# YaqiXia/Voltrix-SpMM

Hardware: AMD Instinct MI355X
Metric: spmm_gflops (higher is better)
Workload: dtype f16

## Files before the change

### voltrix-spmm_amd/voltrix/hybrid.py

```python
from __future__ import annotations

import contextlib
import contextvars
import dataclasses
import os

import torch

from . import capi

DEFAULT_WAVES = 8
DEFAULT_ROW_BLOCKS = 4
DEFAULT_TAU = 3
KSTEP = 32
FUSED_WAVES = 4
FUSED_ROW_BLOCKS = 8


@dataclasses.dataclass
class PanelParts:
    parts: torch.Tensor
    cuts: torch.Tensor
    xcd_ptr: torch.Tensor
    max_parts_per_xcd: int
# ... 11 lines not shown
    panel_order: torch.Tensor
    num_nodes: int
    waves: int
    row_blocks: int
    tau: int
    num_ksteps: int
    num_shared_edges: int
    num_resid_edges: int
    xcd_ptr: torch.Tensor = None
    max_panels_per_xcd: int = 0
    parts: PanelParts = None

    @property
    def panel_rows(self) -> int:
        return self.waves * self.row_blocks * 16

    @property
    def num_panels(self) -> int:
        return (self.num_nodes + self.panel_rows - 1) // self.panel_rows


@dataclasses.dataclass(eq=False)
class TwoLevelHandle:
    blk_offsets: torch.Tensor
    hspa_packed: torch.Tensor
    hind: torch.Tensor
    plan: PanelPlan
    num_nodes: int
    num_edges: int
    hash_tag: str = None
    fused: "FusedRecords" = None
    window_xcd_ptr: torch.Tensor = None
    format_choice: dict = dataclasses.field(default_factory=dict)

    @property
    def residual(self):
        return self.blk_offsets, self.hspa_packed, self.hind


@dataclasses.dataclass
class FusedRecords:
    wave_ptr: torch.Tensor
    records: torch.Tensor
    num_records: int

    def nbytes(self) -> int:
        return self.wave_ptr.numel() * 4 + self.records.numel() * 4


RECORD_WORDS = 64


def build_fused_records_torch(blk_offsets: torch.Tensor, hspa_packed: torch.Tensor, hind: torch.Tensor, num_nodes: int,
                              waves: int = FUSED_WAVES, row_blocks: int = FUSED_ROW_BLOCKS) -> FusedRecords:
    assert blk_offsets.dtype == torch.int32 and hind.dtype == torch.int32 and hspa_packed.dtype == torch.uint32
    device = blk_offsets.device
    num_windows = (num_nodes + 15) // 16
    panel_rows = waves * row_blocks * 16
    num_waves = waves * ((num_nodes + panel_rows - 1) // panel_rows)
    bo = blk_offsets.to(torch.int64)
    kb0, kb1 = bo[:-1], bo[1:]
    nblk = kb1 - kb0
    packed = hspa_packed.view(torch.int32).view(-1, 4)
    hind64 = hind
    total_blocks = packed.shape[0]
    zero_first = (packed[kb0.clamp(max=max(total_blocks - 1, 0))] == 0).all(dim=1) if total_blocks else nblk < 0
# ... 65 lines not shown
    resid_indptr[1:] = torch.cumsum(torch.bincount(resid_rows, minlength=n), 0)
    new_index = torch.cumsum(shared_u.to(torch.int64), 0) - 1
    sk = key[shared_e]
    return (resid_indptr.to(torch.int32), resid_indices, uniq[shared_u], sk % p, new_index[inverse[shared_e]])


MAX_PLAN_COLS = 1 << 22
MAX_PLAN_EDGE_PASSES = 2 * 10 ** 10


def canonical_csr(indptr: torch.Tensor, indices: torch.Tensor, num_nodes: int, num_cols: int):
    deg = (indptr[1:] - indptr[:-1]).to(torch.int64)
    rows = torch.repeat_interleave(torch.arange(num_nodes, device=indptr.device, dtype=torch.int64), deg)
    key = torch.unique(rows * num_cols + indices.to(torch.int64), sorted=True)
    rows = key // num_cols
    out_indptr = torch.zeros(num_nodes + 1, dtype=torch.int64, device=indptr.device)
    out_indptr[1:] = torch.cumsum(torch.bincount(rows, minlength=num_nodes), 0)
    return out_indptr.to(torch.int32), (key - rows * num_cols).to(torch.int32)


def empty_plan(num_nodes, waves, row_blocks, tau, device, num_edges):
    np_ = (num_nodes + waves * row_blocks * 16 - 1) // (waves * row_blocks * 16)
    return PanelPlan(panel_ptr=torch.zeros(np_ + 1, dtype=torch.int32, device=device),
                     panel_cols=torch.zeros(2 * KSTEP, dtype=torch.int32, device=device),
                     panel_bits=torch.zeros(waves * 64, dtype=torch.int32, device=device).view(torch.uint32),
                     panel_order=None, num_nodes=num_nodes, waves=waves, row_blocks=row_blocks, tau=tau, num_ksteps=0,
                     num_shared_edges=0, num_resid_edges=num_edges)


KSTEP_COST_IN_STAGES = 6.6
KSTEP_COST_X10 = 66


def balance_xcd_ranges(two: "TwoLevelHandle") -> None:
    plan = two.plan
    if plan.num_ksteps == 0 or plan.num_panels < 2 * 8:
        return
    cost_x10 = max(1, KSTEP_COST_X10 * plan.panel_rows // 512)
    if plan.panel_ptr.is_cuda:
        xcd_ptr, two.window_xcd_ptr = capi.xcd_ranges_of_panels(plan.panel_ptr, two.blk_offsets, two.num_nodes, plan.panel_rows,
                                                                cost_x10)
    else:
        xcd_ptr, two.window_xcd_ptr = xcd_ranges_of_panels_torch(plan.panel_ptr, two.blk_offsets, two.num_nodes,
                                                                 plan.panel_rows, cost_x10)
    longest_range, longest_panel = torch.stack([(xcd_ptr[1:] - xcd_ptr[:-1]).max(),
                                                (plan.panel_ptr[1:] - plan.panel_ptr[:-1]).max()]).tolist()
    plan.xcd_ptr = xcd_ptr
    plan.max_panels_per_xcd = int(longest_range)
    plan.panel_order = longest_first_order(plan.panel_ptr, xcd_ptr=xcd_ptr)
    cap = default_part_cap(plan.num_ksteps)
    if PANEL_PART_FACTOR > 0 and longest_panel > cap:
        plan.parts = panel_parts(plan.panel_ptr, cap, xcd_ptr)


def xcd_ranges_of_panels_torch(panel_ptr: torch.Tensor, resid_blk_offsets: torch.Tensor, num_nodes: int, panel_rows: int,
                               kstep_cost_x10: int):
    from .schedule import split_equal_work

    dev = panel_ptr.device
    num_panels = panel_ptr.numel() - 1
    windows_per_panel = panel_rows // 16
    num_windows = (num_nodes + 15) // 16
    nst = ((resid_blk_offsets[1:num_windows + 1] - resid_blk_offsets[:num_windows]).to(torch.int64) + 3) // 4
    pad = num_panels * windows_per_panel - num_windows
    stages = torch.cat([nst, torch.zeros(pad, dtype=torch.int64, device=dev)]).view(num_panels, windows_per_panel).sum(1)
    tenths = (panel_ptr[1:] - panel_ptr[:-1]).to(torch.int64) * kstep_cost_x10
    q, r = tenths // 10, tenths % 10
    q = q + ((r > 5) | ((r == 5) & (q % 2 == 1))).to(torch.int64)
    xcd_ptr = split_equal_work(q + stages)
    return xcd_ptr, (xcd_ptr.to(torch.int64) * windows_per_panel).clamp(max=num_windows).to(torch.int32)


PANEL_PART_FACTOR = 1.0
NUM_CUS = 256


def default_part_cap(num_ksteps: int) -> int:
    return max(32, int(PANEL_PART_FACTOR * num_ksteps / NUM_CUS))


def panel_parts(panel_ptr: torch.Tensor, cap: int, panel_xcd_ptr: torch.Tensor = None) -> PanelParts:
    if not panel_ptr.is_cuda:
        return panel_parts_torch(panel_ptr, cap, panel_xcd_ptr)
# ... 142 lines not shown
    bits = torch.zeros((total_ksteps + 1) * waves * 64, dtype=torch.int64, device=device)
    bits.index_add_(0, word, torch.ones_like(word) << (16 * (k % 2) + 4 * j + (k % 8) // 2))
    panel_bits = ((bits + 2 ** 31) % 2 ** 32 - 2 ** 31).to(torch.int32).view(torch.uint32)

    plan = PanelPlan(panel_ptr=panel_ptr.to(torch.int32), panel_cols=panel_cols.to(torch.int32), panel_bits=panel_bits,
                     panel_order=None, num_nodes=num_nodes, waves=waves, row_blocks=row_blocks, tau=tau,
                     num_ksteps=total_ksteps, num_shared_edges=int(rp.numel()),
                     num_resid_edges=int(resid_indices.numel()))
    return resid_indptr, resid_indices, plan


KSTEPS_PIPELINED = 17


def default_panel_tile(embedding_dim: int, waves: int, row_blocks: int = DEFAULT_ROW_BLOCKS):
    if embedding_dim <= 32:
        return (32, 6, 2)
    if embedding_dim <= 64:
        return (64, 6, 2)
    if waves == 8:
        return (128, 3, 1) if row_blocks == 4 else (128, 4, KSTEPS_PIPELINED)
    return (128, 4, 1)


PANEL_DOMINATED_RATIO = 2.0
PANEL_DOMINATED_ROW_BLOCKS = 2


def panel_dominated(plan: "PanelPlan") -> bool:
    resid_stages = max(1.0, plan.num_resid_edges / 32.0)
    return plan.num_ksteps * KSTEP_COST_IN_STAGES >= PANEL_DOMINATED_RATIO * resid_stages


_SIDE_STREAMS = {}


def side_stream(device) -> "torch.cuda.Stream":
    key = device.index if device.index is not None else torch.cuda.current_device()
    if key not in _SIDE_STREAMS:
        _SIDE_STREAMS[key] = torch.cuda.Stream(device=device)
    return _SIDE_STREAMS[key]


def run_two_level(plan: PanelPlan, operand: torch.Tensor, output: torch.Tensor, run_window, out_scale=None,
                  tile=None, concurrent: bool = True) -> None:
    def finish(pending):
        if pending is not None:
            pending.run()

    if plan.num_ksteps == 0:
        finish(run_window(False))
        return
    if not concurrent:
        finish(run_window(False))
        launch_panel(plan, operand, output, accumulate=1, out_scale=out_scale, tile=tile)
        return
    from .utils import timed_launch

    main = torch.cuda.current_stream()
    side = side_stream(operand.device)
    with timed_launch("zero_fill", main):
        output.zero_()
    fork = torch.cuda.Event()
    fork.record(main)
    side.wait_event(fork)
    pending_panel = launch_panel(plan, operand, output, accumulate=2, out_scale=out_scale, tile=tile,
                                 stream=side.cuda_stream, defer_combine=True)
    join = torch.cuda.Event()
    join.record(side)
    pending = run_window(True)
    main.wait_event(join)
    finish(pending)
    finish(pending_panel)


class PendingPanelCombine:

    def __init__(self, plan, partials, output, num_feats, accumulate):
        self.plan, self.partials, self.output, self.num_feats, self.accumulate = plan, partials, output, num_feats, accumulate

    def run(self, raw_stream: int = None):
        from .utils import timed_launch

        current = torch.cuda.current_stream()
        with timed_launch("combine_panel_partials", current) if raw_stream is None else contextlib.nullcontext():
            rc = capi.launch_combine_panel_partials(self.plan.parts, self.partials.data_ptr(), self.output.data_ptr(),
                                                    self.plan.num_nodes, self.num_feats, self.plan.panel_rows,
                                                    self.accumulate, current.cuda_stream if raw_stream is None else raw_stream)
        capi.check(rc, "voltrix_launch_combine_panel_partials")
        self.partials = None


def launch_panel(plan: PanelPlan, feat: torch.Tensor, output: torch.Tensor, accumulate, out_scale=None,
# ... 104 lines not shown
```

### voltrix-spmm_amd/voltrix/include/voltrix/spmm_kernels.hpp

```cpp
#pragma once

#include <hip/hip_runtime.h>

#include <cstdint>
#include <cstdlib>
#include <mutex>
#include <type_traits>
#include <utility>
#include <vector>

#include "voltrix/traits.hpp"

#ifndef VOLTRIX_DIAG
#define VOLTRIX_DIAG 0
#endif


namespace voltrix {

typedef _Float16 half8_t __attribute__((ext_vector_type(8)));
typedef __bf16 bf16x8_t __attribute__((ext_vector_type(8)));
typedef uint16_t bfloat16_bits;
typedef float float4_t __attribute__((ext_vector_type(4)));
typedef unsigned uint2_t __attribute__((ext_vector_type(2)));
// ... 183 lines not shown
    }
  if (hipFuncSetAttribute(kernel, hipFuncAttributeMaxDynamicSharedMemorySize, bytes) != hipSuccess) return kErrBadConfig;
  seen.push_back(Seen{kernel, dev});
  last = seen.back();
  return kOk;
}

template <class T>
struct SpmmArgs {
  using in_t = typename std::conditional<T::EB == 4, float,
                                         typename std::conditional<T::BF16, bfloat16_bits, _Float16>::type>::type;
  const int* blk_offsets;
  const uint32_t* hspa_packed;
  const int* hind;
  const in_t* input;
  float* output;
  int num_nodes;
  int num_windows;
  int F;
  int num_slabs;
  int windows_per_xcd;
  const int* window_order;
  const float* out_scale;
  const int4* units;
  const int* unit_ptr;
  float* partials;
  const in_t* values;
  const int* row_map;
  int slab_major;
  int slab_first;
  int meta_nt;
  int atomic_out;
};

template <int I, int N, class Fn>
__device__ __forceinline__ void static_for(Fn&& fn) {
  if constexpr (I < N) {
    fn(std::integral_constant<int, I>{});
    static_for<I + 1, N>(fn);
  }
}

template <class T, int NU>
__device__ __forceinline__ void spmm_tc16_body(const SpmmArgs<T>& a) {
  static_assert(NU == 1 || NU == 2, "units per wave");
  constexpr int FS = T::FS, D = T::DEPTH, MS = T::META_SLOTS, EB = T::EB;
  constexpr int ROW_BYTES = T::ROW_BYTES, STAGE_BYTES = T::STAGE_BYTES, NDMA = T::DMA_PER_STAGE;
  constexpr int RPD = T::ROWS_PER_DMA, LPR = T::LANES_PER_ROW, SLOTS = T::SLOTS;

  extern __shared__ __attribute__((aligned(16))) char smem[];
  const int lane = threadIdx.x & (kWave - 1);
  const int wave = __builtin_amdgcn_readfirstlane((int)(threadIdx.x / kWave));
  const unsigned long long diag_t0 = (VOLTRIX_DIAG & 8) ? __builtin_amdgcn_s_memrealtime() : 0ull;

  const int xcd = blockIdx.x % kNumXcd;
  int w_begin = xcd * a.windows_per_xcd;
  int w_count = (a.num_windows - w_begin) < a.windows_per_xcd ? (a.num_windows - w_begin) : a.windows_per_xcd;
  if (a.units) {
    w_begin = a.unit_ptr[xcd];
    w_count = a.unit_ptr[xcd + 1] - w_begin;
  }
  __builtin_amdgcn_s_setprio(3);
  const int wave_pos = (int)(blockIdx.x / kNumXcd) * T::WAVES + wave;
  const int pairs_per_slab = (w_count + 1) / 2;
  if (w_count <= 0 || (NU == 1 ? wave_pos >= w_count * a.num_slabs : wave_pos >= pairs_per_slab * a.num_slabs)) return;
  const int lu = NU == 1 ? wave_pos : (wave_pos / pairs_per_slab) * w_count + 2 * (wave_pos % pairs_per_slab);
// ... 340 lines not shown
    wait_vmcnt<0>();
  }

  if (VOLTRIX_DIAG & 4) {
    if (acc[0][0][0] == 12345.678f) a.output[0] = acc[0][0][0];
    return;
  }
  const float oscale = ((EB == 2 && !T::WEIGHTED) ? kAScaleInv : 1.0f) * (a.out_scale ? *a.out_scale : 1.0f);
  const int ocol0 = fs0 + (lane & 15);
#pragma unroll
  for (int p = 0; p < NU; ++p) {
    if (!present[p]) continue;
    const bool dead = NU > 1 && nst_u[p] == 0;
    if (slot[p] >= 0) {
      float* const tile = a.partials + (long long)slot[p] * (kBlkH * (long long)F) + (long long)(4 * (lane >> 4)) * F;
#pragma unroll
      for (int s = 0; s < SLOTS; ++s) {
        const int col = ocol0 + 16 * s;
        if (col < F) {
#pragma unroll
          for (int j = 0; j < 4; ++j) tile[(long long)j * F + col] = dead ? 0.f : acc[p][s][j] * oscale;
        }
      }
      continue;
    }
    const int orow0 = w[p] * kBlkH + 4 * (lane >> 4);
    int orow[4];
#pragma unroll
    for (int j = 0; j < 4; ++j) {
      orow[j] = orow0 + j;
      if (a.row_map && !(VOLTRIX_DIAG & 8)) orow[j] = a.row_map[orow[j]];
      if (orow[j] >= a.num_nodes) orow[j] = -1;
    }
#pragma unroll
    for (int s = 0; s < SLOTS; ++s) {
      const int col = ocol0 + 16 * s;
      if (col < F) {
#pragma unroll
        for (int j = 0; j < 4; ++j) {
          const int row = orow[j];
          if (row >= 0) {
            float* const dst = a.output + ((long long)row * F + col);
            const float v = dead ? 0.f : acc[p][s][j] * oscale;
            if (a.atomic_out)
              unsafeAtomicAdd(dst, v);
            else
              *dst = v;
          }
        }
      }
    }
  }
  if ((VOLTRIX_DIAG & 8) && a.row_map && lane == 0) {
    int* const stamp = const_cast<int*>(a.row_map) + 4ll * ((long long)blockIdx.x * T::WAVES + wave);
    stamp[0] = (int)__builtin_amdgcn_s_getreg((31 << 11) | 20);
    stamp[1] = (int)__builtin_amdgcn_s_getreg((31 << 11) | 4);
    stamp[2] = (int)(unsigned)diag_t0;
    stamp[3] = (int)(unsigned)__builtin_amdgcn_s_memrealtime();
  }
}

template <class T>
static __global__ __launch_bounds__(T::THREADS) void spmm_tc16_kernel(const SpmmArgs<T> a) {
  spmm_tc16_body<T, 1>(a);
}

template <class T>
static __global__ __launch_bounds__(T::THREADS) __attribute__((amdgpu_num_vgpr(160)))
void spmm_tc16_pair_kernel(const SpmmArgs<T> a) {
  spmm_tc16_body<T, 2>(a);
}

inline int slab_major_order(int num_slabs, int slab_row_bytes) { return num_slabs > 1 && slab_row_bytes >= 128; }

enum SlabPolicy : int { kSlabAuto = -1, kSlabOneGrid = 0, kSlabLaunches = 1 };
inline int slab_launch_group(int num_slabs, int slab_row_bytes, long long rows, int policy = kSlabAuto) {
  if (policy == kSlabOneGrid || slab_row_bytes < 128) return 0;
  if (policy == kSlabAuto && rows * 256 > (256ll << 20)) return 0;
  const int group = slab_row_bytes >= 256 ? 1 : 256 / slab_row_bytes;
  return num_slabs > group ? group : 0;
}

template <class T>
inline int launch_spmm_tc16(const int* blk_offsets, const uint32_t* hspa_packed, const int* hind, int num_nodes,
                            int embedding_dim, const void* input ,
                            float* output, hipStream_t stream, const int* window_order = nullptr,
                            const float* out_scale = nullptr, int atomic_out = 0,
                            const int* units = nullptr , const int* unit_ptr = nullptr ,
                            int max_units_per_xcd = 0, float* partials = nullptr, const int* row_map = nullptr,
                            const void* values = nullptr ,
                            int units_per_wave = 1 ,
                            int slab_first = 0, int slab_count = 0 ,
                            long long input_rows = 0 ,
                            int slab_policy = kSlabAuto) {
  if (num_nodes < 0 || embedding_dim < 0) return kErrBadShape;
  if (num_nodes == 0 || embedding_dim == 0) return kOk;
  if (embedding_dim % (16 / T::EB) != 0) return kErrBadShape;
  if (((uintptr_t)input & 15) || ((uintptr_t)hspa_packed & 15)) return kErrBadShape;
  SpmmArgs<T> a;
  a.blk_offsets = blk_offsets;
  a.hspa_packed = hspa_packed;
  a.hind = hind;
  a.input = static_cast<const typename SpmmArgs<T>::in_t*>(input);
  a.output = output;
  a.num_nodes = num_nodes;
  a.num_windows = (num_nodes + kBlkH - 1) / kBlkH;
  a.F = embedding_dim;
  const int total_slabs = (embedding_dim + T::FS - 1) / T::FS;
  if (slab_first < 0 || slab_count < 0 || slab_first + slab_count > total_slabs) return kErrBadShape;
  if (const int group = slab_count == 0 ? slab_launch_group(total_slabs, T::FS * T::EB,
                                                            input_rows > 0 ? input_rows : (long long)num_nodes, slab_policy)
                                        : 0) {
    for (int s = 0; s < total_slabs; s += group) {
      const int rc = launch_spmm_tc16<T>(blk_offsets, hspa_packed, hind, num_nodes, embedding_dim, input, output, stream,
                                         window_order, out_scale, atomic_out, units, unit_ptr, max_units_per_xcd, partials,
                                         row_map, values, units_per_wave, s, total_slabs - s < group ? total_slabs - s : group);
      if (rc != kOk) return rc;
    }
    return kOk;
  }
  a.slab_first = slab_count > 0 ? slab_first : 0;
  a.num_slabs = slab_count > 0 ? slab_count : total_slabs;
  a.windows_per_xcd = (a.num_windows + kNumXcd - 1) / kNumXcd;
  a.window_order = window_order;
  a.out_scale = out_scale;
  a.atomic_out = atomic_out;
  a.meta_nt = total_slabs == 1;
  a.slab_major = slab_major_order(a.num_slabs, T::FS * T::EB);
// ... 309 lines not shown
```

### voltrix-spmm_amd/voltrix/jit_kernels/spmm.py

```python
import contextlib
import contextvars
import ctypes
import os
import warnings
from typing import Callable, NamedTuple

import torch

from ..jit.compiler import hash_to_hex
from ..jit.template import map_ctype
from ..project import TUNE_SPACE_FLAG
from ..schedule import balanced_xcd_windows, default_max_stages, stream_tables, unit_table
from .tuner import jit_tuner

_TUNE_SPACE_OVERRIDE = contextvars.ContextVar("voltrix_tune_space", default=None)


def tune_space_mode() -> str:
    return _TUNE_SPACE_OVERRIDE.get() or os.getenv(TUNE_SPACE_FLAG, "default")


@contextlib.contextmanager
def tune_space(mode: str):
    token = _TUNE_SPACE_OVERRIDE.set(mode)
    try:
        yield
    finally:
        _TUNE_SPACE_OVERRIDE.reset(token)


includes = ('"voltrix/spmm_kernels.hpp"', '"voltrix/spmm_stream_kernels.hpp"')
template = """
if ({SCHED} == 6) {
  __return_code = voltrix::launch_spmm_stream<voltrix::SpmmTile<{FS}, {DEPTH}, {WAVES}, {EB}, {BF16} != 0, {WEIGHTED} != 0>>(
      hspa_packed, hind, num_nodes, embedding_dim, input, output, stream, s_units, s_runs, s_run_ptr, s_max_runs, partials_s,
      out_scale, 0, 0, input_rows, slab_policy);
  if (__return_code == 0 && combine_now != 0)
    __return_code = voltrix::combine_partials(cuts_s, num_cuts_s, partials_s, output, num_nodes, embedding_dim, 0, stream, nullptr);
  return;
}
__return_code = voltrix::launch_spmm_tc16<voltrix::SpmmTile<{FS}, {DEPTH}, {WAVES}, {EB}, {BF16} != 0, {WEIGHTED} != 0>>(
    blk_offsets, hspa_packed, hind,
    num_nodes, embedding_dim, input, output, stream,
    ({SCHED} == 0 || {SCHED} >= 4) ? nullptr : ({SCHED} == 1 ? win_order_a : ({SCHED} == 2 ? win_order_b : win_order_c)),
    out_scale, atomic_out,
    {SCHED} == 4 ? units : ({SCHED} == 5 ? units_p : nullptr), {SCHED} == 5 ? unit_ptr_p : unit_ptr,
    {SCHED} == 5 ? max_units_per_xcd_p : max_units_per_xcd, {SCHED} == 5 ? partials_p : partials,
    has_row_map != 0 ? row_map : nullptr, {WEIGHTED} != 0 ? (const void*)values : nullptr, {SCHED} == 5 ? 2 : 1,
    0, 0, input_rows, slab_policy);
if (__return_code == 0 && {SCHED} == 4 && combine_now != 0)
  __return_code = voltrix::combine_partials(cuts, num_cuts, partials, output, num_nodes, embedding_dim, atomic_out, stream,
                                            has_row_map != 0 ? row_map : nullptr);
if (__return_code == 0 && {SCHED} == 5 && combine_now != 0)
  __return_code = voltrix::combine_partials(cuts_p, num_cuts_p, partials_p, output, num_nodes, embedding_dim, atomic_out,
                                            stream, has_row_map != 0 ? row_map : nullptr);
"""

ORDER_CHUNKS = {1: 128, 2: 512, 3: 2048}
SCHED_UNITS = 4
SCHED_PAIRS = 5
SCHED_STREAM = 6
STREAM_MAX_BLOCKS_PER_WINDOW = 48
PAIR_UNIT_FACTOR = 1.25

SLAB_POLICY = -1


def slab_launches(embedding_dim: int, fs: int, elem_bytes: int, rows: int, policy: int = None) -> int:
    policy = SLAB_POLICY if policy is None else policy
    slabs = -(-embedding_dim // fs)
    slab_bytes = fs * elem_bytes
    if slab_bytes < 128 or policy == 0 or (policy < 0 and rows * 256 > (256 << 20)):
        return 1
    group = 1 if slab_bytes >= 256 else 256 // slab_bytes
    return -(-slabs // group) if slabs > group else 1


def feature_hash(feature: torch.Tensor) -> str:
    if hasattr(feature, "hash_tag") and isinstance(feature.hash_tag, str):
        return hash_to_hex(feature.hash_tag)
    warnings.warn(
        "The feature tensor(i.e. `hspa_packed`)'s hash_tag attr is not set. "
        "Voltrix will use the memory address as the key value for profiling, "
        "which may lead to performance degradation of different cases."
    )
    return hash_to_hex(str(feature.data_ptr()))

# ... 196 lines not shown
        ("win_order_b", torch.int32),
        ("win_order_c", torch.int32),
        ("out_scale", torch.float32),
        ("atomic_out", int),
        ("units", torch.int32),
        ("unit_ptr", torch.int32),
        ("max_units_per_xcd", int),
        ("cuts", torch.int32),
        ("num_cuts", int),
        ("partials", torch.float32),
        ("units_p", torch.int32),
        ("unit_ptr_p", torch.int32),
        ("max_units_per_xcd_p", int),
        ("cuts_p", torch.int32),
        ("num_cuts_p", int),
        ("partials_p", torch.float32),
        ("combine_now", int),
        ("row_map", torch.int32),
        ("has_row_map", int),
        ("values", dtype),
        ("input_rows", int),
        ("slab_policy", int),
        ("s_units", torch.int32),
        ("s_runs", torch.int32),
        ("s_run_ptr", torch.int32),
        ("s_max_runs", int),
        ("cuts_s", torch.int32),
        ("num_cuts_s", int),
        ("partials_s", torch.float32),
        ("stream", torch.cuda.Stream),
    )


def _pair_max_stages(blk_offsets: torch.Tensor, num_nodes: int) -> int:
    return max(8, int(PAIR_UNIT_FACTOR * default_max_stages(blk_offsets, num_nodes) / 1.5))


def handle_unit_table(blk_offsets: torch.Tensor, hspa_packed: torch.Tensor, num_nodes: int, pairs: bool = False,
                      xcd_ptr: torch.Tensor = None):
    def build():
        ranges = xcd_ptr if xcd_ptr is not None else balanced_xcd_windows(blk_offsets, num_nodes)
        return unit_table(blk_offsets, num_nodes, _pair_max_stages(blk_offsets, num_nodes) if pairs else None, xcd_ptr=ranges)

    key = (blk_offsets.data_ptr(), num_nodes, xcd_ptr.data_ptr() if xcd_ptr is not None else 0)
    return _cached_on(hspa_packed, "_voltrix_unit_table_pairs" if pairs else "_voltrix_unit_table", key, build)


def handle_stream_table(blk_offsets: torch.Tensor, hspa_packed: torch.Tensor, hind: torch.Tensor, num_nodes: int):
    return _cached_on(hspa_packed, "_voltrix_stream_table", (blk_offsets.data_ptr(), num_nodes),
                      lambda: stream_tables(blk_offsets, hspa_packed, hind, num_nodes))


def graph_bucket_keys(blk_offsets: torch.Tensor, num_nodes: int, keys: dict):
    import math

    num_windows = (num_nodes + 15) // 16
    if num_windows == 0:
        return None

    def bucket():
        nblk = (blk_offsets[1:num_windows + 1] - blk_offsets[:num_windows]).float()
        sample = nblk[:: max(1, num_windows // (1 << 20))]
        q = torch.quantile(sample, torch.tensor([0.25, 0.5, 0.75], device=nblk.device))
        stats = torch.cat([q, nblk.mean()[None], nblk.std(unbiased=False)[None]]).tolist()

        def half_octave(v):
            return int(round(2 * math.log2(max(v, 1.0))))

        return {"log2_rows": int(round(math.log2(max(num_nodes, 1)))),
                "log2_mean_blocks_x2": half_octave(stats[3]),
                "quartiles_x2": [half_octave(v) for v in stats[:3]],
                "cv_x4": int(round(4 * stats[4] / max(stats[3], 1e-9)))}

    out = {k: v for k, v in keys.items() if k not in ("feature_hash", "device")}
    try:
        out["arch"] = torch.cuda.get_device_properties(blk_offsets.device).gcnArchName.split(":")[0]
    except (AttributeError, RuntimeError):
        out["arch"] = keys.get("device", "unknown")
# ... 23 lines not shown
        from .. import capi

        stream = torch.cuda.current_stream().cuda_stream if stream is None else stream
        rc = capi.launch_combine_partials(self.table, self.partials.data_ptr(), self.output.data_ptr(), self.num_nodes,
                                          self.embedding_dim, self.accumulate, stream,
                                          self.row_map.data_ptr() if self.row_map is not None else 0)
        capi.check(rc, "voltrix_launch_combine_partials")


def _raw_stream(device) -> int:
    try:
        return torch._C._cuda_getCurrentRawStream(device.index if device.index is not None else torch.cuda.current_device())
    except AttributeError:
        return torch.cuda.current_stream(device).cuda_stream


class _TableSchedule(NamedTuple):
    fields: tuple
    partials: str
    handle_table: Callable
    range_table: Callable
    combine_rows: bool

    def launch_args(self, table, embedding_dim, device):
        out = {arg: getattr(table, attr) for arg, attr in self.fields}
        out[self.partials] = torch.empty(max(1, table.num_slots) * 16 * embedding_dim, dtype=torch.float32, device=device)
        return out


_UNIT_FIELDS = ("units", "unit_ptr", "max_units_per_xcd", "cuts", "num_cuts")
TABLE_SCHEDULES = {
    SCHED_UNITS: _TableSchedule(
        tuple(zip(_UNIT_FIELDS, _UNIT_FIELDS)), "partials",
        lambda blk, hspa, hind, n, xcd_ptr: handle_unit_table(blk, hspa, n, xcd_ptr=xcd_ptr),
        lambda blk, hspa, hind, n, full: unit_table(blk, n), combine_rows=True),
    SCHED_PAIRS: _TableSchedule(
        tuple((f + "_p", f) for f in _UNIT_FIELDS), "partials_p",
        lambda blk, hspa, hind, n, xcd_ptr: handle_unit_table(blk, hspa, n, pairs=True, xcd_ptr=xcd_ptr),
        lambda blk, hspa, hind, n, full: unit_table(blk, n, _pair_max_stages(blk, n)), combine_rows=True),
    SCHED_STREAM: _TableSchedule(
        (("s_units", "units"), ("s_runs", "runs"), ("s_run_ptr", "run_ptr"), ("s_max_runs", "max_runs_per_xcd"), ("cuts_s", "cuts"),
         ("num_cuts_s", "num_cuts")), "partials_s",
        lambda blk, hspa, hind, n, xcd_ptr: handle_stream_table(blk, hspa, hind, n),
        lambda blk, hspa, hind, n, full: stream_tables(blk, hspa, hind, n, cut_stages=full.cut_stages), combine_rows=False),
}
_ORDER_ARGS = {1: "win_order_a", 2: "win_order_b", 3: "win_order_c"}


def _pack(arg_defs, named):
    names = [name for name, _ in arg_defs]
    assert named.keys() == set(names), f"missing {set(names) - named.keys()}, unknown {named.keys() - set(names)}"
    return tuple(named[name] for name in names)


_NOT_KEPT = frozenset(("input", "output", "out_scale", "values", "hspa_packed") + tuple(s.partials for s in TABLE_SCHEDULES.values()))


def plan_keepalive(named) -> tuple:
    return tuple(value for name, value in named.items() if name not in _NOT_KEPT and isinstance(value, torch.Tensor))


class _LaunchPlan:
    __slots__ = ("fn", "cargs", "generation", "operand_index", "partials_index", "partials_floats", "combine_table", "combine_args",
                 "device", "keepalive")
    PATCHED = ("input", "output", "out_scale", "values", "stream")

    def launch(self, input, output, out_scale, values, defer_combine):
        i_input, i_output, i_scale, i_values, i_stream = self.operand_index
        cargs = list(self.cargs)
        cargs[i_input] = ctypes.c_void_p(input.data_ptr())
        cargs[i_output] = ctypes.c_void_p(output.data_ptr())
        cargs[i_scale] = ctypes.c_void_p(out_scale.data_ptr())
        cargs[i_values] = ctypes.c_void_p((values if values is not None else input).data_ptr())
        partials = None
        if self.partials_index is not None:
            partials = torch.empty(self.partials_floats, dtype=torch.float32, device=input.device)
            cargs[self.partials_index] = ctypes.c_void_p(partials.data_ptr())
        cargs[i_stream] = ctypes.c_void_p(_raw_stream(self.device))
        rc = ctypes.c_int(-1)
        self.fn(*cargs, ctypes.byref(rc))
        assert rc.value == 0, f"spmm_kernel failed with return code {rc.value}"
        if self.combine_table is not None:
            pending = PendingCombine(self.combine_table, partials, output, *self.combine_args)
            if defer_combine:
                return pending
        return None


def spmm_kernel(blk_offsets, hspa_packed, hind, num_nodes, num_edges, embedding_dim, input, output, out_scale=None,
                atomic_out=False, beside_panel=False, defer_combine=False, row_map=None, values=None, xcd_ptr=None):
    from ..utils import KernelTimer

    plan_key = (blk_offsets.data_ptr(), hind.data_ptr(), num_nodes, embedding_dim, input.dtype, input.shape[0], bool(atomic_out),
                bool(beside_panel), bool(defer_combine), row_map.data_ptr() if row_map is not None else 0,
                values.data_ptr() if values is not None else 0, xcd_ptr.data_ptr() if xcd_ptr is not None else 0,
                getattr(hspa_packed, "hash_tag", None), tune_space_mode(), SLAB_POLICY)
    plans = getattr(hspa_packed, "_voltrix_plans", None)
    plan = plans.get(plan_key) if plans is not None else None
    if plan is not None and plan.generation == jit_tuner.generation and KernelTimer.active is None:
        assert input.is_contiguous() and output.is_contiguous() and input.shape[1] == embedding_dim
        assert output.shape[0] == num_nodes and output.shape[1] == embedding_dim and output.dtype == torch.float32
        return plan.launch(input, output, out_scale if out_scale is not None else unit_scale(input.device), values, defer_combine)

    assert blk_offsets.is_cuda and blk_offsets.dtype == torch.int32
    assert hspa_packed.is_cuda and hspa_packed.dtype == torch.uint32
    assert hind.is_cuda and hind.dtype == torch.int32
    assert input.is_cuda and input.dtype in (torch.float, torch.float16, torch.bfloat16) and input.is_contiguous()
    assert output.is_cuda and output.dtype == torch.float and output.is_contiguous()
    assert input.dim() == 2 and input.shape[1] == embedding_dim
    assert output.shape[0] == num_nodes and output.shape[1] == embedding_dim
    elem_bytes = input.element_size()
    assert embedding_dim % (16 // elem_bytes) == 0, "embedding_dim must keep rows 16-byte aligned (voltrix.spmm pads)"
    if out_scale is None:
        out_scale = unit_scale(input.device)
    assert out_scale.is_cuda and out_scale.dtype == torch.float32 and out_scale.numel() >= 1
    if row_map is not None:
        assert row_map.is_cuda and row_map.dtype == torch.int32 and row_map.numel() == 16 * ((num_nodes + 15) // 16)

    if values is not None:
        assert values.is_cuda and values.dtype == input.dtype and elem_bytes == 2 and values.is_contiguous()
        assert values.numel() * 4 == hspa_packed.numel() * 128, "value plane: 128 values per TC block"
    short_windows = hspa_packed.numel() // 4 <= STREAM_MAX_BLOCKS_PER_WINDOW * ((num_nodes + 15) // 16)
    space = tile_space(embedding_dim, elem_bytes, input.dtype == torch.bfloat16,
                       TWO_LEVEL_LDS_BUDGET if beside_panel else None, weighted=values is not None,
                       stream_ok=not atomic_out and row_map is None and (short_windows or tune_space_mode() == "stream"),
                       shallow_ok=short_windows)
    keys = {
        "feature_hash": feature_hash(hspa_packed),
        "embedding_dim": embedding_dim,
        "dtype": str(input.dtype),
        "device": torch.cuda.get_device_name(input.device),
        "two_level": bool(beside_panel),
        "weighted": values is not None,
    }
    if row_map is not None:
        keys["row_map"] = True
    chosen = jit_tuner.tuned_point("spmm_kernel", keys).get("SCHED") if jit_tuner.is_tuned("spmm_kernel", keys) else None
    tables = {sched: desc.handle_table(blk_offsets, hspa_packed, hind, num_nodes, xcd_ptr) for sched, desc in TABLE_SCHEDULES.items()
              if (chosen == sched if chosen is not None else any(p["SCHED"] == sched for p in space))}
    needs_orders = chosen is None or chosen in ORDER_CHUNKS

    def orders(blk, n):
        return {arg: window_order(blk, hspa_packed, n, sched) if needs_orders else blk for sched, arg in _ORDER_ARGS.items()}

    arg_defs = arg_defs_for(input.dtype)
    named = dict(blk_offsets=blk_offsets, hspa_packed=hspa_packed, hind=hind, num_nodes=num_nodes, num_edges=num_edges,
                 embedding_dim=embedding_dim, input=input, output=output, **orders(blk_offsets, num_nodes), out_scale=out_scale,
                 atomic_out=int(bool(atomic_out)), combine_now=int(not defer_combine),
                 row_map=row_map if row_map is not None else blk_offsets, has_row_map=int(row_map is not None),
                 values=values if values is not None else input, input_rows=int(input.shape[0]), slab_policy=int(SLAB_POLICY),
                 stream=torch.cuda.current_stream())
    types = dict(arg_defs)
    for sched, desc in TABLE_SCHEDULES.items():
        if sched in tables:
            named.update(desc.launch_args(tables[sched], embedding_dim, input.device))
        else:
            named.update({arg: 0 if types[arg] is int else blk_offsets for arg, _ in desc.fields}, **{desc.partials: out_scale})
    args = _pack(arg_defs, named)
    tune_named = named
    if len(space) > 1 and chosen is None and (atomic_out or defer_combine):
        tune_named = dict(named, output=torch.zeros_like(output) if atomic_out else output, combine_now=1)
    tune_args = _pack(arg_defs, tune_named)

    def sample_args():
        num_windows = (num_nodes + 15) // 16
        ranges = sample_ranges(num_windows, int(blk_offsets[num_windows]))
        if len(ranges) == 1 and ranges[0] == (0, num_windows):
            return [tune_args], 1.0
        out_full = tune_named["output"]
        launches, covered = [], 0
        for w0, w1 in ranges:
            sub = blk_offsets[w0:w1 + 1]
            n_sub = min(num_nodes, 16 * w1) - 16 * w0
            covered += w1 - w0
            a = dict(tune_named, blk_offsets=sub, num_nodes=n_sub, **orders(sub, n_sub),
                     output=out_full if row_map is not None else out_full[16 * w0:16 * w0 + n_sub],
                     combine_now=1)
            for sched, table in tables.items():
                desc = TABLE_SCHEDULES[sched]
                a.update(desc.launch_args(desc.range_table(sub, hspa_packed, hind, n_sub, table), embedding_dim, input.device))
            if row_map is not None:
                a["row_map"] = row_map[16 * w0:16 * w1]
            launches.append(_pack(arg_defs, a))
        return launches, covered / max(1, num_windows)

    staged = tune_space_mode() != "full"

    def tune(use_store=True):
        return jit_tuner.compile_and_tune(
            name="spmm_kernel", keys=keys, space=space, includes=includes, arg_defs=arg_defs, template=template, args=tune_args,
            kernel_tag="spmm", bench=sweep_bench, bucket_keys=lambda: graph_bucket_keys(blk_offsets, num_nodes, keys),
            use_store=use_store, sample_args=sample_args, stages=sweep_stages if staged else None, budget_s=sweep_budget_s)

    runtime = tune()
    rc = runtime(*args)
    signature = jit_tuner._signature("spmm_kernel", keys)
    if rc != 0 and signature in jit_tuner.unvalidated:
        jit_tuner.forget("spmm_kernel", keys)
        runtime = tune(use_store=False)
        rc = runtime(*args)
    jit_tuner.unvalidated.discard(signature)
    assert rc == 0, f"spmm_kernel failed with return code {rc}"
    sched = jit_tuner.tuned_point("spmm_kernel", keys).get("SCHED")
    table = tables.get(sched)
    combine_args = None
    if defer_combine and table is not None and table.num_cuts > 0:
        combine_args = (num_nodes, embedding_dim) + ((bool(atomic_out), row_map) if TABLE_SCHEDULES[sched].combine_rows else (False, None))
    fn, kernel_args = runtime.launcher()
    names = [name for name, _ in kernel_args]
    plan = _LaunchPlan()
    plan.fn, plan.generation, plan.device = fn, jit_tuner.generation, input.device
    plan.cargs = [map_ctype(named[name]) for name in names]
    plan.operand_index = tuple(names.index(name) for name in _LaunchPlan.PATCHED)
    plan.keepalive = plan_keepalive(named) + tuple(tables.values()) + ((xcd_ptr,) if xcd_ptr is not None else ())
    has_partials = table is not None and table.num_slots > 0
    plan.partials_index = names.index(TABLE_SCHEDULES[sched].partials) if has_partials else None
    plan.partials_floats = table.num_slots * 16 * embedding_dim if has_partials else 0
    plan.combine_table, plan.combine_args = (table, combine_args) if combine_args is not None else (None, None)
    try:
        if plans is None:
            plans = hspa_packed._voltrix_plans = {}
        plans[plan_key] = plan
    except AttributeError:
        pass
    if combine_args is not None:
        return PendingCombine(table, named[TABLE_SCHEDULES[sched].partials], output, *combine_args)
    return None
```

### voltrix-spmm_amd/voltrix/project/const.py

```python
PROJECT_NAME_FULL = "Voltrix-SpMM"
PROJECT_NAME_ABBR = "Voltrix"
PROJECT_NAME_FULL_LOWER = "voltrix-spmm"
PROJECT_NAME_ABBR_LOWER = "voltrix"

DEBUG_FLAG = "VOLTRIX_JIT_DEBUG"
NVCC_COMPILER_FLAG = "VOLTRIX_NVCC_COMPILER"
CACHE_DIR_FLAG = "VOLTRIX_CACHE_DIR"
PTXAS_VERBOSE_FLAG = "VOLTRIX_PTXAS_VERBOSE"
JIT_PRINT_NVCC_COMMAND_FLAG = "VOLTRIX_JIT_PRINT_NVCC_COMMAND"
PRINT_AUTOTUNE_FLAG = "VOLTRIX_PRINT_AUTO_TUNE"

HIPCC_COMPILER_FLAG = "VOLTRIX_HIPCC_COMPILER"
FP32_MODE_FLAG = "VOLTRIX_FP32_MODE"
PREPROCESS_FLAG = "VOLTRIX_PREPROCESS"
TUNE_SPACE_FLAG = "VOLTRIX_TUNE_SPACE"
TUNED_STORE_FLAG = "VOLTRIX_TUNED_STORE"
TUNED_DEFAULTS_FLAG = "VOLTRIX_TUNED_DEFAULTS"
HYBRID_FLAG = "VOLTRIX_HYBRID"
HYBRID_MIN_SHARE_FLAG = "VOLTRIX_HYBRID_MIN_SHARE"
FUSED_FLAG = "VOLTRIX_FUSED"
CSR_PATH_FLAG = "VOLTRIX_CSR_PATH"
SUPPORTED_FLAGS = (DEBUG_FLAG, NVCC_COMPILER_FLAG, CACHE_DIR_FLAG, PTXAS_VERBOSE_FLAG, JIT_PRINT_NVCC_COMMAND_FLAG,
                   PRINT_AUTOTUNE_FLAG, HIPCC_COMPILER_FLAG, FP32_MODE_FLAG, PREPROCESS_FLAG, TUNE_SPACE_FLAG,
                   TUNED_STORE_FLAG, TUNED_DEFAULTS_FLAG, HYBRID_FLAG, HYBRID_MIN_SHARE_FLAG, FUSED_FLAG, CSR_PATH_FLAG)
```

### voltrix-spmm_amd/voltrix/spmm/spmm.py

```python
import math
import os

import torch

from ..jit_kernels import (
    csr_fused_preprocess_kernel,
    hmat_gen_kernel,
    hmat_packed_swizzle_kernel,
    preprocess_kernel,
    spmm_kernel,
)
from .. import capi, hybrid, sidecar
from ..project import CSR_PATH_FLAG, FP32_MODE_FLAG, PREPROCESS_FLAG

BLK_H = 16
BLK_W = 8


def csr_preprocess(indptr: torch.Tensor, indices: torch.Tensor, num_nodes: int, num_cols: int = None):
    assert indptr.is_cpu and indptr.dtype == torch.int32
    assert indices.is_cpu and indices.dtype == torch.int32
    assert indptr.numel() == num_nodes + 1

    if preprocess_mode()[0] != "reference":
# ... 284 lines not shown
    signature = ("spmm_format", f"{{'device': '{torch.cuda.get_device_name(hspa_packed.device)}', 'dtype': '{key[1]}', "
                                f"'embedding_dim': {key[0]}, 'feature_hash': '{feature_hash(hspa_packed)}'}}")
    stored = jit_tuner._load_store().get(f"{signature[0]}|{signature[1]}")
    if stored in ("two-level", "window") and hasattr(hspa_packed, "hash_tag"):
        return stored
    times = {}
    for name, fn in (("window", window), ("two-level", two_level)):
        fn()
        start, end = torch.cuda.Event(enable_timing=True), torch.cuda.Event(enable_timing=True)
        start.record()
        for _ in range(3):
            fn()
        end.record()
        end.synchronize()
        times[name] = start.elapsed_time(end)
    best = min(times, key=times.get)
    if os.getenv("VOLTRIX_PRINT_AUTO_TUNE") or os.getenv("VOLTRIX_JIT_DEBUG"):
        print(f"voltrix.spmm format for width {key[0]} {key[1]}: {times} -> {best}")
    if hasattr(hspa_packed, "hash_tag"):
        jit_tuner._save_choice(signature, best)
    return best


def _run_two_level(two, operand, output, out_scale, tag_source=None, concurrent=True):
    if two.fused is not None and hybrid.fused_enabled():
        hybrid.launch_fused(two.plan, two.fused, operand, output, out_scale=out_scale)
        return
    resid = two.hspa_packed
    if getattr(resid, "hash_tag", None) is None:
        tag = two.hash_tag or getattr(tag_source, "hash_tag", None)
        if isinstance(tag, str):
            resid.hash_tag = tag + "/residual"

    def run_window(atomic):
        return spmm_kernel(two.blk_offsets, resid, two.hind, num_nodes=two.num_nodes,
                           num_edges=two.plan.num_resid_edges, embedding_dim=operand.shape[1], input=operand,
                           output=output, out_scale=out_scale, atomic_out=atomic,
                           beside_panel=two.plan.num_ksteps > 0, defer_combine=True, xcd_ptr=two.window_xcd_ptr)

    hybrid.run_two_level(two.plan, operand, output, run_window, out_scale=out_scale, concurrent=concurrent)


def spmm_two_level(handle: "hybrid.TwoLevelHandle", feat: torch.Tensor, concurrent: bool = True):
    assert isinstance(handle, hybrid.TwoLevelHandle)
    num_feats = feat.shape[1]
    operand, out_scale, padded, exact = _operand(feat)
    assert not (exact and handle.plan.num_ksteps > 0), \
        "the panel kernel takes a 16-bit operand (unset VOLTRIX_FP32_MODE=exact or use csr_preprocess)"
    output = torch.empty((handle.num_nodes, padded), dtype=torch.float32, device=feat.device)
    _run_two_level(handle, operand, output, out_scale, concurrent=concurrent)
    return output if padded == num_feats else output[:, :num_feats].contiguous()
```

Before: 21430.

## Split two-level SpMM into row halves to avoid zero-fill and atomic joins

Adds a 'halves' join mode that splits panels into two row ranges balanced by window stages against panel k-steps. The panel kernel on the side stream and the window kernel on the main stream each take one half first with plain stores, then add onto the other half with a new non-atomic read-add-store output mode. This removes the full output zero-fill and the atomic adds from the concurrent path, at the cost of extra events, cross-stream dependencies and a second read of the output for the add phase. It applies only to large outputs with narrow operands and is on by default.

```diff
diff --git a/voltrix-spmm_amd/voltrix/hybrid.py b/voltrix-spmm_amd/voltrix/hybrid.py
--- a/voltrix-spmm_amd/voltrix/hybrid.py
+++ b/voltrix-spmm_amd/voltrix/hybrid.py
@@ -67,6 +67,7 @@
     fused: "FusedRecords" = None
     window_xcd_ptr: torch.Tensor = None
     format_choice: dict = dataclasses.field(default_factory=dict)
+    join_halves: object = None
 
     @property
     def residual(self):
@@ -198,7 +199,7 @@
 KSTEP_COST_X10 = 66
 
 
-def balance_xcd_ranges(two: "TwoLevelHandle") -> None:
+def balance_xcd_ranges(two: "TwoLevelHandle", part_ksteps: int = None) -> None:
     plan = two.plan
     if plan.num_ksteps == 0 or plan.num_panels < 2 * 8:
         return
@@ -214,7 +215,7 @@
     plan.xcd_ptr = xcd_ptr
     plan.max_panels_per_xcd = int(longest_range)
     plan.panel_order = longest_first_order(plan.panel_ptr, xcd_ptr=xcd_ptr)
-    cap = default_part_cap(plan.num_ksteps)
+    cap = default_part_cap(plan.num_ksteps if part_ksteps is None else part_ksteps)
     if PANEL_PART_FACTOR > 0 and longest_panel > cap:
         plan.parts = panel_parts(plan.panel_ptr, cap, xcd_ptr)
 
@@ -423,6 +424,87 @@
     return plan.num_ksteps * KSTEP_COST_IN_STAGES >= PANEL_DOMINATED_RATIO * resid_stages
 
 
+JOIN_HALVES_MIN_OUTPUT_BYTES = 16 << 20
+
+def join_mode() -> str:
+    v = os.getenv("VOLTRIX_JOIN", "halves")
+    assert v in ("halves", "atomic"), f"VOLTRIX_JOIN={v}"
+    return v
+
+
+def choose_split(stages, ksteps) -> int:
+    stages, ksteps = [int(v) for v in stages], [int(v) for v in ksteps]
+    assert len(stages) == len(ksteps)
+    with_ksteps = [p for p, k in enumerate(ksteps) if k > 0]
+    if len(with_ksteps) < 2:
+        return 0
+    total_k = sum(ksteps)
+    if sum(stages) == 0:
+        stages = ksteps
+    total_s = sum(stages)
+    first, last = with_ksteps[0], with_ksteps[-1]
+    below = sum(stages[:first + 1])
+    above = total_k - sum(ksteps[:first + 1])
+    best, best_gap = 0, None
+    for b in range(first + 1, last + 1):
+        gap = abs(below * total_k - above * total_s)
+        if best_gap is None or gap < best_gap:
+            best, best_gap = b, gap
+        below += stages[b]
+        above -= ksteps[b]
+    return best
+
+
+@dataclasses.dataclass(eq=False)
+class JoinHalf:
+    handle: "TwoLevelHandle"
+    row0: int
+    panel0: int
+
+
+def panel_work(two: "TwoLevelHandle"):
+    plan = two.plan
+    num_windows = (two.num_nodes + 15) // 16
+    wpp = plan.panel_rows // 16
+    nst = ((two.blk_offsets[1:num_windows + 1] - two.blk_offsets[:num_windows]).to(torch.int64) + 3) // 4
+    pad = torch.zeros(plan.num_panels * wpp - num_windows, dtype=torch.int64, device=nst.device)
+    stages = torch.cat([nst, pad]).view(plan.num_panels, wpp).sum(1)
+    ksteps = (plan.panel_ptr[1:] - plan.panel_ptr[:-1]).to(torch.int64)
+    stages, ksteps = torch.stack([stages, ksteps]).tolist()
+    return stages, ksteps
+
+
+def build_join_halves(two: "TwoLevelHandle"):
+    plan = two.plan
+    stages, ksteps = panel_work(two)
+    b = choose_split(stages, ksteps)
+    if b == 0:
+        return False
+    num_windows = (two.num_nodes + 15) // 16
+    wpp = plan.panel_rows // 16
+    halves = []
+    for p0, p1 in ((0, b), (b, plan.num_panels)):
+        row0 = p0 * plan.panel_rows
+        rows = min(two.num_nodes, p1 * plan.panel_rows) - row0
+        w0, w1 = p0 * wpp, min(num_windows, p1 * wpp)
+        sub_plan = dataclasses.replace(plan, panel_ptr=plan.panel_ptr[p0:p1 + 1], num_nodes=rows, num_ksteps=sum(ksteps[p0:p1]),
+                                       panel_order=None, xcd_ptr=None, max_panels_per_xcd=0, parts=None)
+        sub_plan.panel_order = longest_first_order(sub_plan.panel_ptr)
+        sub = TwoLevelHandle(two.blk_offsets[w0:w1 + 1], two.hspa_packed, two.hind, sub_plan, rows, two.num_edges)
+        balance_xcd_ranges(sub, part_ksteps=plan.num_ksteps)
+        halves.append(JoinHalf(sub, row0, p0))
+    return tuple(halves)
+
+
+def join_halves_of(two: "TwoLevelHandle", operand: torch.Tensor, output: torch.Tensor):
+    if (join_mode() != "halves" or two.plan.num_ksteps == 0 or operand.shape[1] * operand.element_size() > 256
+            or output.numel() * output.element_size() < JOIN_HALVES_MIN_OUTPUT_BYTES):
+        return None
+    if two.join_halves is None:
+        two.join_halves = build_join_halves(two)
+    return two.join_halves or None
+
+
 _SIDE_STREAMS = {}
 
 
@@ -434,7 +516,7 @@
 
 
 def run_two_level(plan: PanelPlan, operand: torch.Tensor, output: torch.Tensor, run_window, out_scale=None,
-                  tile=None, concurrent: bool = True) -> None:
+                  tile=None, concurrent: bool = True, halves=None) -> None:
     def finish(pending):
         if pending is not None:
             pending.run()
@@ -450,6 +532,38 @@
 
     main = torch.cuda.current_stream()
     side = side_stream(operand.device)
+    if halves is not None:
+        from .jit_kernels.spmm import OUT_ADD, OUT_STORE
+
+        lo, hi = halves
+        keep = []
+
+        def panel(half, accumulate):
+            rows = output[half.row0:half.row0 + half.handle.num_nodes]
+            pending_panel = launch_panel(half.handle.plan, operand, rows, accumulate=accumulate, out_scale=out_scale, tile=tile,
+                                         stream=side.cuda_stream, defer_combine=True)
+            if pending_panel is not None:
+                keep.append(pending_panel.partials)
+                pending_panel.run(side.cuda_stream)
+
+        fork = torch.cuda.Event()
+        fork.record(main)
+        side.wait_event(fork)
+        panel(hi, 0)
+        p_hi = torch.cuda.Event()
+        p_hi.record(side)
+        finish(run_window(OUT_STORE, lo))
+        w_lo = torch.cuda.Event()
+        w_lo.record(main)
+        side.wait_event(w_lo)
+        panel(lo, 1)
+        join = torch.cuda.Event()
+        join.record(side)
+        main.wait_event(p_hi)
+        finish(run_window(OUT_ADD, hi))
+        main.wait_event(join)
+        del keep
+        return
     with timed_launch("zero_fill", main):
         output.zero_()
     fork = torch.cuda.Event()
diff --git a/voltrix-spmm_amd/voltrix/include/voltrix/spmm_kernels.hpp b/voltrix-spmm_amd/voltrix/include/voltrix/spmm_kernels.hpp
--- a/voltrix-spmm_amd/voltrix/include/voltrix/spmm_kernels.hpp
+++ b/voltrix-spmm_amd/voltrix/include/voltrix/spmm_kernels.hpp
@@ -239,6 +239,8 @@
   int meta_nt;
   int atomic_out;
 };
+enum OutMode : int { kOutStore = 0, kOutAtomic = 1, kOutAdd = 2 };
+constexpr int kAddSlots = 4;
 
 template <int I, int N, class Fn>
 __device__ __forceinline__ void static_for(Fn&& fn) {
@@ -645,6 +647,31 @@
       if (a.row_map && !(VOLTRIX_DIAG & 8)) orow[j] = a.row_map[orow[j]];
       if (orow[j] >= a.num_nodes) orow[j] = -1;
     }
+    if (a.atomic_out == kOutAdd) {
+      constexpr int AS = SLOTS < kAddSlots ? SLOTS : kAddSlots;
+#pragma unroll
+      for (int s0 = 0; s0 < SLOTS; s0 += AS) {
+        float prev[AS][4];
+#pragma unroll
+        for (int s = 0; s < AS; ++s) {
+          const int col = ocol0 + 16 * (s0 + s);
+#pragma unroll
+          for (int j = 0; j < 4; ++j)
+            prev[s][j] = (col < F && orow[j] >= 0) ? a.output[(long long)orow[j] * F + col] : 0.f;
+        }
+#pragma unroll
+        for (int s = 0; s < AS; ++s) {
+          const int col = ocol0 + 16 * (s0 + s);
+          if (col < F) {
+#pragma unroll
+            for (int j = 0; j < 4; ++j)
+              if (orow[j] >= 0)
+                a.output[(long long)orow[j] * F + col] = prev[s][j] + (dead ? 0.f : acc[p][s0 + s][j] * oscale);
+          }
+        }
+      }
+      continue;
+    }
 #pragma unroll
     for (int s = 0; s < SLOTS; ++s) {
       const int col = ocol0 + 16 * s;
@@ -655,7 +682,7 @@
           if (row >= 0) {
             float* const dst = a.output + ((long long)row * F + col);
             const float v = dead ? 0.f : acc[p][s][j] * oscale;
-            if (a.atomic_out)
+            if (a.atomic_out == kOutAtomic)
               unsafeAtomicAdd(dst, v);
             else
               *dst = v;
@@ -706,7 +733,7 @@
                             int slab_first = 0, int slab_count = 0 ,
                             long long input_rows = 0 ,
                             int slab_policy = kSlabAuto) {
-  if (num_nodes < 0 || embedding_dim < 0) return kErrBadShape;
+  if (num_nodes < 0 || embedding_dim < 0 || atomic_out < kOutStore || atomic_out > kOutAdd) return kErrBadShape;
   if (num_nodes == 0 || embedding_dim == 0) return kOk;
   if (embedding_dim % (16 / T::EB) != 0) return kErrBadShape;
   if (((uintptr_t)input & 15) || ((uintptr_t)hspa_packed & 15)) return kErrBadShape;
diff --git a/voltrix-spmm_amd/voltrix/jit_kernels/spmm.py b/voltrix-spmm_amd/voltrix/jit_kernels/spmm.py
--- a/voltrix-spmm_amd/voltrix/jit_kernels/spmm.py
+++ b/voltrix-spmm_amd/voltrix/jit_kernels/spmm.py
@@ -49,10 +49,10 @@
     has_row_map != 0 ? row_map : nullptr, {WEIGHTED} != 0 ? (const void*)values : nullptr, {SCHED} == 5 ? 2 : 1,
     0, 0, input_rows, slab_policy);
 if (__return_code == 0 && {SCHED} == 4 && combine_now != 0)
-  __return_code = voltrix::combine_partials(cuts, num_cuts, partials, output, num_nodes, embedding_dim, atomic_out, stream,
+  __return_code = voltrix::combine_partials(cuts, num_cuts, partials, output, num_nodes, embedding_dim, atomic_out != 0, stream,
                                             has_row_map != 0 ? row_map : nullptr);
 if (__return_code == 0 && {SCHED} == 5 && combine_now != 0)
-  __return_code = voltrix::combine_partials(cuts_p, num_cuts_p, partials_p, output, num_nodes, embedding_dim, atomic_out,
+  __return_code = voltrix::combine_partials(cuts_p, num_cuts_p, partials_p, output, num_nodes, embedding_dim, atomic_out != 0,
                                             stream, has_row_map != 0 ? row_map : nullptr);
 """
 
@@ -315,18 +315,25 @@
     )
 
 
+OUT_STORE, OUT_ATOMIC, OUT_ADD = 0, 1, 2
+
+
 def _pair_max_stages(blk_offsets: torch.Tensor, num_nodes: int) -> int:
     return max(8, int(PAIR_UNIT_FACTOR * default_max_stages(blk_offsets, num_nodes) / 1.5))
 
 
 def handle_unit_table(blk_offsets: torch.Tensor, hspa_packed: torch.Tensor, num_nodes: int, pairs: bool = False,
-                      xcd_ptr: torch.Tensor = None):
+                      xcd_ptr: torch.Tensor = None, whole=None):
     def build():
         ranges = xcd_ptr if xcd_ptr is not None else balanced_xcd_windows(blk_offsets, num_nodes)
-        return unit_table(blk_offsets, num_nodes, _pair_max_stages(blk_offsets, num_nodes) if pairs else None, xcd_ptr=ranges)
+        bound = _pair_max_stages(*(whole or (blk_offsets, num_nodes))) if pairs else (default_max_stages(*whole) if whole else None)
+        return unit_table(blk_offsets, num_nodes, bound, xcd_ptr=ranges)
 
     key = (blk_offsets.data_ptr(), num_nodes, xcd_ptr.data_ptr() if xcd_ptr is not None else 0)
-    return _cached_on(hspa_packed, "_voltrix_unit_table_pairs" if pairs else "_voltrix_unit_table", key, build)
+    attr = "_voltrix_unit_table_pairs" if pairs else "_voltrix_unit_table"
+    if whole is not None:
+        attr += f"_{key[0]:x}_{num_nodes}"
+    return _cached_on(hspa_packed, attr, key, build)
 
 
 def handle_stream_table(blk_offsets: torch.Tensor, hspa_packed: torch.Tensor, hind: torch.Tensor, num_nodes: int):
@@ -416,16 +423,16 @@
 TABLE_SCHEDULES = {
     SCHED_UNITS: _TableSchedule(
         tuple(zip(_UNIT_FIELDS, _UNIT_FIELDS)), "partials",
-        lambda blk, hspa, hind, n, xcd_ptr: handle_unit_table(blk, hspa, n, xcd_ptr=xcd_ptr),
+        lambda blk, hspa, hind, n, xcd_ptr, whole=None: handle_unit_table(blk, hspa, n, xcd_ptr=xcd_ptr, whole=whole),
         lambda blk, hspa, hind, n, full: unit_table(blk, n), combine_rows=True),
     SCHED_PAIRS: _TableSchedule(
         tuple((f + "_p", f) for f in _UNIT_FIELDS), "partials_p",
-        lambda blk, hspa, hind, n, xcd_ptr: handle_unit_table(blk, hspa, n, pairs=True, xcd_ptr=xcd_ptr),
+        lambda blk, hspa, hind, n, xcd_ptr, whole=None: handle_unit_table(blk, hspa, n, pairs=True, xcd_ptr=xcd_ptr, whole=whole),
         lambda blk, hspa, hind, n, full: unit_table(blk, n, _pair_max_stages(blk, n)), combine_rows=True),
     SCHED_STREAM: _TableSchedule(
         (("s_units", "units"), ("s_runs", "runs"), ("s_run_ptr", "run_ptr"), ("s_max_runs", "max_runs_per_xcd"), ("cuts_s", "cuts"),
          ("num_cuts_s", "num_cuts")), "partials_s",
-        lambda blk, hspa, hind, n, xcd_ptr: handle_stream_table(blk, hspa, hind, n),
+        lambda blk, hspa, hind, n, xcd_ptr, whole=None: handle_stream_table(blk, hspa, hind, n),
         lambda blk, hspa, hind, n, full: stream_tables(blk, hspa, hind, n, cut_stages=full.cut_stages), combine_rows=False),
 }
 _ORDER_ARGS = {1: "win_order_a", 2: "win_order_b", 3: "win_order_c"}
@@ -472,10 +479,13 @@
 
 
 def spmm_kernel(blk_offsets, hspa_packed, hind, num_nodes, num_edges, embedding_dim, input, output, out_scale=None,
-                atomic_out=False, beside_panel=False, defer_combine=False, row_map=None, values=None, xcd_ptr=None):
+                atomic_out=False, beside_panel=False, defer_combine=False, row_map=None, values=None, xcd_ptr=None,
+                bucket_of=None):
     from ..utils import KernelTimer
 
-    plan_key = (blk_offsets.data_ptr(), hind.data_ptr(), num_nodes, embedding_dim, input.dtype, input.shape[0], bool(atomic_out),
+    atomic_out = int(atomic_out)
+    assert atomic_out in (OUT_STORE, OUT_ATOMIC, OUT_ADD), atomic_out
+    plan_key = (blk_offsets.data_ptr(), hind.data_ptr(), num_nodes, embedding_dim, input.dtype, input.shape[0], atomic_out,
                 bool(beside_panel), bool(defer_combine), row_map.data_ptr() if row_map is not None else 0,
                 values.data_ptr() if values is not None else 0, xcd_ptr.data_ptr() if xcd_ptr is not None else 0,
                 getattr(hspa_packed, "hash_tag", None), tune_space_mode(), SLAB_POLICY)
@@ -520,7 +530,7 @@
     if row_map is not None:
         keys["row_map"] = True
     chosen = jit_tuner.tuned_point("spmm_kernel", keys).get("SCHED") if jit_tuner.is_tuned("spmm_kernel", keys) else None
-    tables = {sched: desc.handle_table(blk_offsets, hspa_packed, hind, num_nodes, xcd_ptr) for sched, desc in TABLE_SCHEDULES.items()
+    tables = {sched: desc.handle_table(blk_offsets, hspa_packed, hind, num_nodes, xcd_ptr, bucket_of) for sched, desc in TABLE_SCHEDULES.items()
               if (chosen == sched if chosen is not None else any(p["SCHED"] == sched for p in space))}
     needs_orders = chosen is None or chosen in ORDER_CHUNKS
 
@@ -530,7 +540,7 @@
     arg_defs = arg_defs_for(input.dtype)
     named = dict(blk_offsets=blk_offsets, hspa_packed=hspa_packed, hind=hind, num_nodes=num_nodes, num_edges=num_edges,
                  embedding_dim=embedding_dim, input=input, output=output, **orders(blk_offsets, num_nodes), out_scale=out_scale,
-                 atomic_out=int(bool(atomic_out)), combine_now=int(not defer_combine),
+                 atomic_out=atomic_out, combine_now=int(not defer_combine),
                  row_map=row_map if row_map is not None else blk_offsets, has_row_map=int(row_map is not None),
                  values=values if values is not None else input, input_rows=int(input.shape[0]), slab_policy=int(SLAB_POLICY),
                  stream=torch.cuda.current_stream())
@@ -573,7 +583,8 @@
     def tune(use_store=True):
         return jit_tuner.compile_and_tune(
             name="spmm_kernel", keys=keys, space=space, includes=includes, arg_defs=arg_defs, template=template, args=tune_args,
-            kernel_tag="spmm", bench=sweep_bench, bucket_keys=lambda: graph_bucket_keys(blk_offsets, num_nodes, keys),
+            kernel_tag="spmm", bench=sweep_bench,
+            bucket_keys=lambda: graph_bucket_keys(*(bucket_of if bucket_of is not None else (blk_offsets, num_nodes)), keys),
             use_store=use_store, sample_args=sample_args, stages=sweep_stages if staged else None, budget_s=sweep_budget_s)
 
     runtime = tune()
@@ -586,6 +597,7 @@
     jit_tuner.unvalidated.discard(signature)
     assert rc == 0, f"spmm_kernel failed with return code {rc}"
     sched = jit_tuner.tuned_point("spmm_kernel", keys).get("SCHED")
+    assert not (atomic_out and sched == SCHED_STREAM), "the stream kernel stores: it cannot add onto the output"
     table = tables.get(sched)
     combine_args = None
     if defer_combine and table is not None and table.num_cuts > 0:
diff --git a/voltrix-spmm_amd/voltrix/project/const.py b/voltrix-spmm_amd/voltrix/project/const.py
--- a/voltrix-spmm_amd/voltrix/project/const.py
+++ b/voltrix-spmm_amd/voltrix/project/const.py
@@ -20,6 +20,7 @@
 HYBRID_MIN_SHARE_FLAG = "VOLTRIX_HYBRID_MIN_SHARE"
 FUSED_FLAG = "VOLTRIX_FUSED"
 CSR_PATH_FLAG = "VOLTRIX_CSR_PATH"
+JOIN_FLAG = "VOLTRIX_JOIN"
 SUPPORTED_FLAGS = (DEBUG_FLAG, NVCC_COMPILER_FLAG, CACHE_DIR_FLAG, PTXAS_VERBOSE_FLAG, JIT_PRINT_NVCC_COMMAND_FLAG,
                    PRINT_AUTOTUNE_FLAG, HIPCC_COMPILER_FLAG, FP32_MODE_FLAG, PREPROCESS_FLAG, TUNE_SPACE_FLAG,
-                   TUNED_STORE_FLAG, TUNED_DEFAULTS_FLAG, HYBRID_FLAG, HYBRID_MIN_SHARE_FLAG, FUSED_FLAG, CSR_PATH_FLAG)
+                   TUNED_STORE_FLAG, TUNED_DEFAULTS_FLAG, HYBRID_FLAG, HYBRID_MIN_SHARE_FLAG, FUSED_FLAG, CSR_PATH_FLAG, JOIN_FLAG)
diff --git a/voltrix-spmm_amd/voltrix/spmm/spmm.py b/voltrix-spmm_amd/voltrix/spmm/spmm.py
--- a/voltrix-spmm_amd/voltrix/spmm/spmm.py
+++ b/voltrix-spmm_amd/voltrix/spmm/spmm.py
@@ -340,13 +340,17 @@
         if isinstance(tag, str):
             resid.hash_tag = tag + "/residual"
 
-    def run_window(atomic):
-        return spmm_kernel(two.blk_offsets, resid, two.hind, num_nodes=two.num_nodes,
+    def run_window(atomic, half=None):
+        h = two if half is None else half.handle
+        rows = output if half is None else output[half.row0:half.row0 + h.num_nodes]
+        return spmm_kernel(h.blk_offsets, resid, two.hind, num_nodes=h.num_nodes,
                            num_edges=two.plan.num_resid_edges, embedding_dim=operand.shape[1], input=operand,
-                           output=output, out_scale=out_scale, atomic_out=atomic,
-                           beside_panel=two.plan.num_ksteps > 0, defer_combine=True, xcd_ptr=two.window_xcd_ptr)
-
-    hybrid.run_two_level(two.plan, operand, output, run_window, out_scale=out_scale, concurrent=concurrent)
+                           output=rows, out_scale=out_scale, atomic_out=atomic,
+                           beside_panel=two.plan.num_ksteps > 0, defer_combine=True, xcd_ptr=h.window_xcd_ptr,
+                           bucket_of=None if half is None else (two.blk_offsets, two.num_nodes))
+
+    halves = hybrid.join_halves_of(two, operand, output) if concurrent else None
+    hybrid.run_two_level(two.plan, operand, output, run_window, out_scale=out_scale, concurrent=concurrent, halves=halves)
 
 
 def spmm_two_level(handle: "hybrid.TwoLevelHandle", feat: torch.Tensor, concurrent: bool = True):
```

Measured after the change: 18720. 12.7% lower.
